# gabinsane/multimodal-vae-comparison

Measured on AMD Instinct MI355X. Metric: training samples/sec, MoPoE CdSprites+ L2 (fwd+bwd+Adam), higher is better.
Workload: dtype f32; 1 GPU; configs[1]: MoPoE, CdSprites+ L2 shapes, CNN2 image tower + TxtTransformer text tower, n_latents=32, batch=128/GPU, T=32; Adam(amsgrad) lr 1e-4, beta 1, train mode (dropout on); global_batch=128, parallelism=dp1, settle_steps=40

## Files before the change

include/mmvae_hip.h:

```cpp
#ifndef MMVAE_HIP_H
#define MMVAE_HIP_H

#include <stddef.h>
#include <stdint.h>

#ifdef __cplusplus
extern "C" {
#endif

typedef void* mmvae_stream_t;

enum {
  MMVAE_OK = 0,
  MMVAE_ERR_ARG = 1,
  MMVAE_ERR_UNSUPPORTED = 2,
  MMVAE_ERR_LAUNCH = 3
};

enum { MMVAE_ACT_NONE = 0, MMVAE_ACT_SILU = 1, MMVAE_ACT_RELU = 2, MMVAE_ACT_GELU = 3 };
enum {
  MMVAE_EP_NONE = 0,
  MMVAE_EP_RELU = 1,
  MMVAE_EP_MUL_RELU_MASK = 2,
  MMVAE_EP_MUL_SILU_GRAD = 3,
// ... 45 lines not shown
                           const mmvae_dropout_t* drop, const mmvae_dropout_t* ln_drop, mmvae_stream_t stream);
int mmvae_ffn32_bwd_b16(const float* x, const float* dy, const void* wsplit, const float* b1, float* dx, float* ws,
                        void* rsplit, const float* dx_add, int M, int FF, const mmvae_dropout_t* drop,
                        mmvae_stream_t stream);

int mmvae_version(void);
const char* mmvae_arch(void);


int mmvae_conv2d_k4s2_fwd(const float* x, const float* w, const float* bias, const float* aux, float* y,
                          int B, int Cin, int Cout, int Hin, int in_act, int ep_mode, mmvae_stream_t stream);

int mmvae_conv2d_k4s2_dgrad(const float* dy, const float* w, const float* aux, float* dx,
                            int B, int Cin, int Cout, int Hout, int ep_mode, mmvae_stream_t stream);

int mmvae_conv2d_k4s2_wgrad(const float* dy, const float* x, float* dw, float* db, float* ws,
                            int B, int Cin, int Cout, int Hout, int x_act, int accumulate, mmvae_stream_t stream);

int mmvae_convT2d_k4s2_fwd(const float* x, const float* w, const float* bias, const float* aux, float* y,
                           int B, int Cin, int Cout, int Hin, int in_act, int ep_mode, mmvae_stream_t stream);

int mmvae_convT2d_k4s2_dgrad(const float* dy, const float* w, const float* aux, float* dx,
                             int B, int Cin, int Cout, int Hin, int ep_mode, mmvae_stream_t stream);

int mmvae_convT2d_k4s2_wgrad(const float* x, const float* dy, float* dw, float* db, float* ws,
                             int B, int Cin, int Cout, int Hin, int x_act, int accumulate, mmvae_stream_t stream);

size_t mmvae_conv_wgrad_ws_floats(int B, int Csmall, int Clarge, int Hsmall);

int mmvae_conv2d_k4s2_bwd(const float* dy, const float* x, const float* w, float* dx, float* dw, float* db, float* ws,
                          int B, int Cin, int Cout, int Hout, int x_act, int accumulate, mmvae_stream_t stream);
int mmvae_convT2d_k4s2_bwd(const float* dy, const float* x, const float* w, float* dx, float* dw, float* db, float* ws,
                           int B, int Cin, int Cout, int Hin, int x_act, int accumulate, mmvae_stream_t stream);
int mmvae_convT3_bce_seeded(const float* x, const float* w, const float* bias, const float* target, float* row,
                            float* dlogit, float* part, unsigned* ticket, int B, int in_act, float seed,
                            mmvae_stream_t stream);
int mmvae_convT3_bce_strips(int B);
int mmvae_conv_plan(int split_bf16);

int mmvae_gemm_f32(const float* A, const float* Bm, const float* bias, const float* aux, float* C,
                   float* a_rowsum, float* ws, int M, int N, int K, long sam, long sak, long sbk, long sbn,
                   long ldc, int a_act, int b_act, int ep_mode, int accumulate, int splitk,
                   mmvae_stream_t stream);
size_t mmvae_gemm_ws_floats(int M, int N, int splitk);
int mmvae_gemm_splits(int M, int N, int K, int splitk);
int mmvae_gemm_b16_set(int on);
int mmvae_bias_group_add(float* y, const float* bias, int rows, int C, int G, mmvae_stream_t stream);
size_t mmvae_bias_group_ws_floats(int rows, int C);
int mmvae_bias_group_parts(int rows);
int mmvae_bias_group_grad(const float* dy, float* db, float* ws, int rows, int C, int G, int accumulate,
                          mmvae_stream_t stream);

int mmvae_linear_fwd(const float* x, const float* w, const float* b, float* aux, float* y, int M, int N, int K,
                     long ldx, int x_act, int ep_mode, mmvae_stream_t stream);
int mmvae_linear_bwd_data(const float* dy, const float* w, const float* aux, float* dx, int M, int N, int K,
                          int ep_mode, int accumulate, mmvae_stream_t stream);
int mmvae_linear_bwd_weight(const float* dy, const float* x, float* dw, float* db, float* ws, int M, int N, int K,
                            long ldx, int x_act, int accumulate, mmvae_stream_t stream);
size_t mmvae_linear_bwd_weight_ws_floats(int M, int N, int K);
#define MMVAE_WGRAD_BATCH_MAX 8
typedef struct {
  const float* dy; const float* x; float* dw; float* db; float* ws;
  int M, N, K; long ldx; int x_act, accumulate;
} mmvae_wgrad_job_t;
int mmvae_linear_bwd_weight_batch(const mmvae_wgrad_job_t* jobs, int n_jobs, mmvae_stream_t stream);
typedef struct {
// ... 487 lines not shown
```

multimodal_vae_comparison_amd/csrc/conv.hip:

```cpp
#include "conv_common.hpp"

#include "conv_gather.inc"
#include "conv_gather_b16.inc"
#include "conv_scatter.inc"
#include "conv_scatter_b16.inc"
#include "conv_wgrad.inc"

constexpr int cmax(int a, int b) { return a > b ? a : b; }

template <typename G, typename W, bool SPEC = false>
__global__ __launch_bounds__(256) void conv2d_bwd_fused_kernel(ConvScatterArgs ad, ConvWgradArgs aw, int n_w, int w_gx) {
  MMVAE_TRACE_STAMP(10 + G::LGH);
  __shared__ __attribute__((aligned(16))) float smem[cmax(G::SMEM, W::SMEM)];
  if ((int)blockIdx.x < n_w) conv_wgrad_body<W, SPEC>(aw, blockIdx.x % w_gx, blockIdx.x / w_gx, w_gx, smem);
  else
    conv_scatter_body<G>(ad, (n_w & 7) ? (int)blockIdx.x - n_w : xcd_contiguous(blockIdx.x - n_w, gridDim.x - n_w), smem);
}
template <typename G, typename W, bool SPEC = false>
__global__ __launch_bounds__(256) void convT_bwd_fused_kernel(ConvGatherArgs ad, ConvWgradArgs aw, int n_w, int w_gx) {
  MMVAE_TRACE_STAMP(14 - G::LGH);
  __shared__ __attribute__((aligned(16))) float smem[cmax(G::SMEM, W::SMEM)];
  if ((int)blockIdx.x < n_w) conv_wgrad_body<W, SPEC>(aw, blockIdx.x % w_gx, blockIdx.x / w_gx, w_gx, smem);
  else
    conv_gather_body<G, G::RWONLY>(ad, (n_w & 7) ? (int)blockIdx.x - n_w : xcd_contiguous(blockIdx.x - n_w, gridDim.x - n_w),
                                   smem);
}

template <typename GS, typename W, bool SPEC = false>
__global__ __launch_bounds__(256) void conv2d_bwd_fused_b16_kernel(ConvScatterArgs ad, ConvWgradArgs aw, int n_w, int w_gx) {
  MMVAE_TRACE_STAMP(10 + GS::LGH);
  __shared__ __attribute__((aligned(16))) unsigned char smem[cmax(GS::SMEM_TOTAL, 4 * W::SMEM)];
  if ((int)blockIdx.x < n_w)
    conv_wgrad_body<W, SPEC>(aw, blockIdx.x % w_gx, blockIdx.x / w_gx, w_gx, reinterpret_cast<float*>(smem));
  else
    conv_scatter_b16_body<GS, MMVAE_ACT_NONE>(
        ad, (n_w & 7) ? (int)blockIdx.x - n_w : xcd_contiguous(blockIdx.x - n_w, gridDim.x - n_w), 0, smem);
}

template <typename GB, typename W, bool SPEC = false>
__global__ __launch_bounds__(256) void convT_bwd_fused_b16_kernel(ConvGatherArgs ad, ConvWgradArgs aw, int n_w, int w_gx) {
  MMVAE_TRACE_STAMP(14 - GB::LGH);
  __shared__ __attribute__((aligned(16))) unsigned char smem[cmax(GB::SMEM_TOTAL, 4 * W::SMEM)];
  if ((int)blockIdx.x < n_w)
    conv_wgrad_body<W, SPEC>(aw, blockIdx.x % w_gx, blockIdx.x / w_gx, w_gx, reinterpret_cast<float*>(smem));
  else
    conv_gather_b16p_body<GB, MMVAE_ACT_NONE>(
        ad, (n_w & 7) ? (int)blockIdx.x - n_w : xcd_contiguous(blockIdx.x - n_w, gridDim.x - n_w), 0, smem);
}

// ... 43 lines not shown
        hipLaunchKernelGGL((conv2d_bwd_fused_b16_kernel<GS, W, true>), dim3(n_w + n_d), dim3(256), 0, st, ad, aw, n_w, nsplit);
      else
        hipLaunchKernelGGL((conv2d_bwd_fused_b16_kernel<GS, W>), dim3(n_w + n_d), dim3(256), 0, st, ad, aw, n_w, nsplit);
    };
    if (wgrad_qc8(nsplit, n_macro)) go(WgradGeom<32, 4, 8>{});
    else go(WgradGeom<32, 4>{});
    int rc0 = mmvae_launch_status();
    if (rc0) return rc0;
    return conv_bwd_reduce(ws, dw, db, B, Cin, Hout, 32, accumulate, stream);
  }
  scatter_visit(Hout, scatter_plan(tiles, 32, Hout), [&](auto g) {
    using G = decltype(g);
    if constexpr (G::LGH <= 4) {
      const int n_d = (int)scatter_grid(B, Hout, G::TM);
      if (wgrad_qc8(nsplit, n_macro)) {
        using W = WgradGeom<32, G::LGH, 8>;
        const int n_w = nsplit * W::NCH;
        if (wgrad_spec(n_macro, nsplit))
          hipLaunchKernelGGL((conv2d_bwd_fused_kernel<G, W, true>), dim3(n_w + n_d), dim3(256), 0, st, ad, aw, n_w, nsplit);
        else
          hipLaunchKernelGGL((conv2d_bwd_fused_kernel<G, W>), dim3(n_w + n_d), dim3(256), 0, st, ad, aw, n_w, nsplit);
      } else {
        using W = WgradGeom<32, G::LGH>;
        const int n_w = nsplit * W::NCH;
        hipLaunchKernelGGL((conv2d_bwd_fused_kernel<G, W>), dim3(n_w + n_d), dim3(256), 0, st, ad, aw, n_w, nsplit);
      }
      launched = true;
    }
  });
  if (!launched) return MMVAE_ERR_UNSUPPORTED;
  int rc = mmvae_launch_status();
  if (rc) return rc;
  return conv_bwd_reduce(ws, dw, db, B, Cin, Hout, 32, accumulate, stream);
}

extern "C" int mmvae_convT2d_k4s2_bwd(const float* dy, const float* x, const float* w, float* dx, float* dw, float* db,
                                      float* ws, int B, int Cin, int Cout, int Hin, int x_act, int accumulate,
                                      mmvae_stream_t stream) {
  MMVAE_CHECK_ARG(dy && x && w && dx && dw && ws && B > 0);
  hipStream_t st = (hipStream_t)stream;
  const int ep = dact_ep(x_act);
  const bool fused = Cin == 32 && (Cout == 32 || Cout == 3) && Hin >= 4 && Hin <= 32 && !(Hin & (Hin - 1)) &&
                     !(Cout == 3 && Hin != 32) && !(Cout == 32 && Hin > 16);
  if (!fused) {
    int rc = conv_wgrad_dispatch(x, dy, dw, db, ws, B, Cin, Cout, Hin, x_act, MMVAE_ACT_NONE, db ? 2 : 0, accumulate, st);
    if (rc) return rc;
    return conv_gather_dispatch(dy, w, nullptr, x, dx, B, Cout, Cin, 2 * Hin, MMVAE_ACT_NONE, ep, st);
  }
  ConvGatherArgs ad{dy, w, nullptr, x, dx, B, MMVAE_ACT_NONE, ep, CONV_CO};
  const long tiles = ((long)B * Hin * Hin + 31) / 32;
  const int n_macro = wgrad_n_macro(B, Hin), nsplit = wgrad_splits(n_macro, Cout);
  ConvWgradArgs aw{x, dy, ws, B, x_act, MMVAE_ACT_NONE, db ? 2 : 0, n_macro, 32, (long)32 * Cout * 16 + 32};
  bool launched = false;
  auto b16 = [&](auto gb) {
    using GB = decltype(gb);
    const int n_d = (int)((long)B * GB::HOUT / GB::NR);
    auto go = [&](auto wg) {
      using W = decltype(wg);
      const int n_w = nsplit * W::NCH;
      if (wgrad_spec(n_macro, nsplit))
        hipLaunchKernelGGL((convT_bwd_fused_b16_kernel<GB, W, true>), dim3(n_w + n_d), dim3(256), 0, st, ad, aw, n_w, nsplit);
      else
        hipLaunchKernelGGL((convT_bwd_fused_b16_kernel<GB, W>), dim3(n_w + n_d), dim3(256), 0, st, ad, aw, n_w, nsplit);
    };
    if constexpr (GB::CIN == 32) {
      if (wgrad_qc8(nsplit, n_macro)) go(WgradGeom<32, GB::LGH - 1, 8>{});
// ... 112 lines not shown
```

multimodal_vae_comparison_amd/csrc/conv_scatter.inc:

```
#include "conv_common.hpp"

struct ConvScatterArgs {
  const float* x;
  const float* w;
  const float* bias;
  const float* aux;
  float* y;
  int B, in_act, ep;
  int co_total;
};

template <int LGH_, int TM_, int CC_, int CIN_ = 32>
struct ScatterGeom {
  static constexpr int CIN = CIN_, LGH = LGH_, TM = TM_, CC = CC_;
  static constexpr int HIN = 1 << LGH, WIN = HIN, HOUT = 2 * HIN, WOUT = HOUT, LGW = LGH;
  static constexpr int RPT = WIN >= 32 ? 1 : 32 / WIN;
  static constexpr int NR = TM * RPT;
  static constexpr int NIMG = NR <= HIN ? 1 : NR / HIN;
  static constexpr int NROW = NR <= HIN ? NR : HIN;
  static constexpr int NRIN = NROW + 2;
  static constexpr int C0 = 4;
  static constexpr int RS = WIN == 16 ? 48 : WIN == 8 ? 40 : WIN == 4 ? 36 : 40;
  static constexpr int CS = NRIN * RS;
  static constexpr int IS0 = CC * CS;
  static constexpr int IS = (WIN == 4 && NIMG > 1) ? IS0 + ((16 - IS0 % 32 + 32) % 32) : IS0;
  static constexpr int KS = 4 / TM, CPW = CC / KS, NCHUNK = CIN / CC;
  static constexpr int RAW = NIMG * IS;
  static constexpr int IN_FLOATS = (KS > 1 && RAW < 4096) ? 4096 : (RAW + 3) / 4 * 4;
  static constexpr int SMEM = IN_FLOATS + CC * 16 * CONV_CO;
  static constexpr int F4ROW = WIN / 4, F4PP = NRIN * F4ROW;
  static constexpr int NF4 = NIMG * CC * F4PP;
  static constexpr int NSLOT = (NF4 + 255) / 256;
  static constexpr int WSLOT = CC * 4 * CONV_CO / 256;
  static_assert(CIN % CC == 0 && CC % KS == 0 && TM * KS == 4, "tile shape");
  static_assert(NSLOT <= 32, "validity mask");
};

template <typename G>
__device__ __forceinline__ void conv_scatter_body(const ConvScatterArgs& a, const int bid_x, float* __restrict__ smem,
                                                  const int og = 0) {
  constexpr int CIN = G::CIN, TM = G::TM, CC = G::CC, KS = G::KS, CPW = G::CPW;
  constexpr int HIN = G::HIN, WIN = G::WIN, HOUT = G::HOUT, WOUT = G::WOUT, LGW = G::LGW;
  constexpr int RS = G::RS, CS = G::CS;
  float* __restrict__ s_in = smem;
  float* __restrict__ s_w = smem + G::IN_FLOATS;

  const int tid = threadIdx.x, lane = tid & 63, wave = __builtin_amdgcn_readfirstlane(tid >> 6);
  const int li = lane & 31, lh = lane >> 5;
  const int tm = wave % TM, ks = wave / TM;
  const int Mtot = a.B * HIN * WIN;
  const int first_row = bid_x * G::NR;
  const int b0 = first_row >> LGW;
  const int h0 = G::NIMG > 1 ? 0 : first_row & (HIN - 1);

  int goff[G::NSLOT], lpos[G::NSLOT];
  unsigned svalid = 0;
#pragma unroll
  for (int s = 0; s < G::NSLOT; ++s) {
    const int q = tid + 256 * s;
    const int plane = q / G::F4PP, f = q - plane * G::F4PP;
    const int lr = f / G::F4ROW, c4 = f - lr * G::F4ROW;
    const int img = plane / CC, c = plane - img * CC;
    const int ih = h0 - 1 + lr;
    const bool ok = q < G::NF4 && ih >= 0 && ih < HIN && (b0 + img) < a.B;
    svalid |= (ok ? 1u : 0u) << s;
    goff[s] = ok ? ((img * CIN + c) * HIN + ih) * WIN + 4 * c4 : 0;
    lpos[s] = img * G::IS + c * CS + lr * RS + G::C0 + 4 * c4;
  }
  const float* xbase = a.x + (size_t)b0 * CIN * HIN * WIN;
  float4 rv[G::NSLOT], rw[G::WSLOT];
  auto load_chunk = [&](int ch) {
    const float* xch = xbase + (size_t)ch * CC * HIN * WIN;
#pragma unroll
// ... 12 lines not shown
      for (int s = 0; s < G::NSLOT; ++s) {
        rv[s].x = dev_silu(rv[s].x); rv[s].y = dev_silu(rv[s].y);
        rv[s].z = dev_silu(rv[s].z); rv[s].w = dev_silu(rv[s].w);
      }
    } else if (a.in_act == MMVAE_ACT_RELU) {
#pragma unroll
      for (int s = 0; s < G::NSLOT; ++s) {
        rv[s].x = fmaxf(rv[s].x, 0.f); rv[s].y = fmaxf(rv[s].y, 0.f);
        rv[s].z = fmaxf(rv[s].z, 0.f); rv[s].w = fmaxf(rv[s].w, 0.f);
      }
    }
#pragma unroll
    for (int s = 0; s < G::NSLOT; ++s) {
      if (tid + 256 * s < G::NF4) {
        const bool ok = svalid >> s & 1u;
        float4 o;
        o.x = ok ? rv[s].x : 0.f; o.y = ok ? rv[s].y : 0.f; o.z = ok ? rv[s].z : 0.f; o.w = ok ? rv[s].w : 0.f;
        *reinterpret_cast<float4*>(s_in + lpos[s]) = o;
      }
    }
#pragma unroll
    for (int i = 0; i < G::WSLOT; ++i) {
      const int e4 = i * 256 + tid;
      const int o = e4 & 31, kh = (e4 >> 5) & 3, cl = e4 >> 7;
      const int ph = 1 - (kh & 1), th = kh >> 1;
      float* d0 = s_w + ((((ph * 2 + 0) * CC + cl) * 2 + th) * 2) * CONV_CO + o;
      float* d1 = s_w + ((((ph * 2 + 1) * CC + cl) * 2 + th) * 2) * CONV_CO + o;
      d1[0] = rw[i].x;
      d0[0] = rw[i].y;
      d1[CONV_CO] = rw[i].z;
      d0[CONV_CO] = rw[i].w;
    }
  };

  load_chunk(0);
  for (int i = tid; i < G::NIMG * CC * G::NRIN * 2; i += 256) {
    const int side = i & 1, r = i >> 1;
    const int plane = r / G::NRIN, lr = r - plane * G::NRIN;
    const int img = plane / CC, c = plane - img * CC;
    s_in[img * G::IS + c * CS + lr * RS + G::C0 - 1 + side * (WIN + 1)] = 0.f;
  }

  const int tile_p0 = (bid_x * TM + tm) * 32;
  int abase;
  {
    int p = tile_p0 + li;
    if (p > Mtot - 1) p = Mtot - 1;
    const int R = p >> LGW, s = p & (WIN - 1);
    int rl = R - first_row;
    if (rl < 0) rl = 0;
    const int img_l = G::NIMG > 1 ? rl >> LGW : 0;
    const int r_l = G::NIMG > 1 ? rl & (HIN - 1) : rl;
    abase = img_l * G::IS + (r_l + 1) * RS + (s + G::C0 - lh) + ks * CPW * CS;
  }
  const int wbase = (ks * CPW * 4 + lh) * CONV_CO + li;

  f32x16 acc[4];
#pragma unroll
  for (int c = 0; c < 4; ++c)
#pragma unroll
    for (int r = 0; r < 16; ++r) acc[c][r] = 0.f;

#pragma unroll 1
  for (int ch = 0; ch < G::NCHUNK; ++ch) {
    if (ch > 0) __syncthreads();
    store_chunk();
    __syncthreads();
    if (ch + 1 < G::NCHUNK) load_chunk(ch + 1);
    {
      float av[2][6], bv[2][8];
      auto load_ops = [&](int cc, int buf) {
#pragma unroll
        for (int dr = 0; dr < 3; ++dr)
#pragma unroll
          for (int pw = 0; pw < 2; ++pw) av[buf][dr * 2 + pw] = s_in[abase + cc * CS + (dr - 1) * RS + pw];
#pragma unroll
        for (int cls = 0; cls < 4; ++cls)
#pragma unroll
          for (int th = 0; th < 2; ++th) bv[buf][cls * 2 + th] = s_w[wbase + (((cls * CC + cc) * 2 + th) * 2) * CONV_CO];
      };
      load_ops(0, 0);
#pragma unroll
      for (int cc = 0; cc < CPW; ++cc) {
        if (cc + 1 < CPW) load_ops(cc + 1, (cc + 1) & 1);
        __builtin_amdgcn_sched_barrier(0);
#pragma unroll
        for (int cls = 0; cls < 4; ++cls)
#pragma unroll
          for (int th = 0; th < 2; ++th) {
            const int ph = cls >> 1, pw = cls & 1;
            acc[cls] = __builtin_amdgcn_mfma_f32_32x32x2f32(av[cc & 1][(ph - th + 1) * 2 + pw], bv[cc & 1][cls * 2 + th],
                                                            acc[cls], 0, 0, 0);
          }
        __builtin_amdgcn_sched_barrier(0);
      }
    }
  }

  const float bias = a.bias ? a.bias[og * CONV_CO + li] : 0.f;
  auto store8 = [&](int q, int ph, const float* e0, const float* e1) {
    const int p0 = tile_p0 + 8 * q + 4 * lh;
    if (p0 < Mtot) {
      const int R = p0 >> LGW, s = p0 & (WIN - 1);
      const int b = R >> LGW, r = R & (HIN - 1);
      const size_t off = (((size_t)b * a.co_total + og * CONV_CO + li) * HOUT + 2 * r + ph) * WOUT + 2 * s;
      float4 o0 = make_float4(e0[0] + bias, e1[0] + bias, e0[1] + bias, e1[1] + bias);
      float4 o1 = make_float4(e0[2] + bias, e1[2] + bias, e0[3] + bias, e1[3] + bias);
      if (a.ep != MMVAE_EP_NONE) {
        float4 a0 = make_float4(0.f, 0.f, 0.f, 0.f), a1 = a0;
        if (ep_reads_aux(a.ep)) {
          a0 = *reinterpret_cast<const float4*>(a.aux + off);
          a1 = *reinterpret_cast<const float4*>(a.aux + off + 4);
        }
        o0.x = conv_epilogue(o0.x, a0.x, a.ep); o0.y = conv_epilogue(o0.y, a0.y, a.ep);
        o0.z = conv_epilogue(o0.z, a0.z, a.ep); o0.w = conv_epilogue(o0.w, a0.w, a.ep);
        o1.x = conv_epilogue(o1.x, a1.x, a.ep); o1.y = conv_epilogue(o1.y, a1.y, a.ep);
        o1.z = conv_epilogue(o1.z, a1.z, a.ep); o1.w = conv_epilogue(o1.w, a1.w, a.ep);
      }
      *reinterpret_cast<float4*>(a.y + off) = o0;
      *reinterpret_cast<float4*>(a.y + off + 4) = o1;
    }
  };

  if (KS == 1) {
#pragma unroll
    for (int ph = 0; ph < 2; ++ph)
#pragma unroll
      for (int q = 0; q < 4; ++q) {
        float e0[4], e1[4];
#pragma unroll
        for (int e = 0; e < 4; ++e) {
          e0[e] = acc[ph * 2 + 0][4 * q + e];
          e1[e] = acc[ph * 2 + 1][4 * q + e];
        }
        store8(q, ph, e0, e1);
      }
  } else {
    float* red = s_in;
#pragma unroll
    for (int ph = 0; ph < 2; ++ph) {
      float sum[2][4 / KS][4];
#pragma unroll
      for (int pw = 0; pw < 2; ++pw) {
        __syncthreads();
#pragma unroll
        for (int r = 0; r < 16; ++r) red[(wave * 16 + r) * 64 + lane] = acc[ph * 2 + pw][r];
        __syncthreads();
#pragma unroll
        for (int qq = 0; qq < 4 / KS; ++qq) {
          const int q = ks * (4 / KS) + qq;
#pragma unroll
          for (int e = 0; e < 4; ++e) {
            float s = 0.f;
#pragma unroll
            for (int k2 = 0; k2 < KS; ++k2) s += red[((k2 * TM + tm) * 16 + 4 * q + e) * 64 + lane];
            sum[pw][qq][e] = s;
          }
        }
      }
#pragma unroll
      for (int qq = 0; qq < 4 / KS; ++qq) store8(ks * (4 / KS) + qq, ph, sum[0][qq], sum[1][qq]);
    }
  }
}

struct ConvScatter3Args {
  const float* x;
  const float* w;
  const float* bias;
  float* y;
  int B, in_act, ep;
};

template <int LGH_, int NT_ = 2>
struct Scatter3Geom {
  static constexpr int CIN = 32, CO = 3, LGH = LGH_;
  static constexpr int NT = NT_;
  static constexpr int POS = 64 * NT;
  static constexpr int HIN = 1 << LGH, WIN = HIN, HOUT = 2 * HIN, WOUT = HOUT;
  static constexpr int NR = POS / WIN;
  static constexpr int NRIN = NR + 2;
  static constexpr int C0 = 4;
  static constexpr int RS = (WIN + 5 + 3) / 4 * 4;
  static constexpr int CS0 = NRIN * RS;
  static constexpr int CS = CS0 + ((16 - CS0 % 32 + 32) % 32);
  static constexpr int IN_FLOATS = CIN * CS;
  static constexpr int SMEM = IN_FLOATS + 9 * CIN * 16;
  static constexpr int F4ROW = WIN / 4, F4PP = NRIN * F4ROW, NF4 = CIN * F4PP, NSLOT = (NF4 + 255) / 256;
  static_assert(NR >= 1 && NR <= HIN, "one image per workgroup");
};

template <typename G>
__device__ __forceinline__ void conv_scatter3_body(const ConvScatter3Args& a, const int bid_x, float* __restrict__ smem) {
  constexpr int CIN = G::CIN, CO = G::CO, HIN = G::HIN, WIN = G::WIN, HOUT = G::HOUT, WOUT = G::WOUT;
  constexpr int RS = G::RS, CS = G::CS;
// ... 210 lines not shown
```

multimodal_vae_comparison_amd/hipops.py:

```python
import ctypes
import os

import torch

_HERE = os.path.dirname(os.path.abspath(__file__))
LIB_PATH = os.path.join(_HERE, "libmmvae_hip.so")
_lib = None

c_p = ctypes.c_void_p
c_i = ctypes.c_int
c_l = ctypes.c_long
c_f = ctypes.c_float
c_u = ctypes.c_uint
c_sz = ctypes.c_size_t

MAX_EXPERTS = 8

ACT_NONE, ACT_SILU, ACT_RELU, ACT_GELU = 0, 1, 2, 3
EP_NONE, EP_RELU, EP_MUL_RELU_MASK, EP_MUL_SILU_GRAD, EP_GELU, EP_MUL_GELU_GRAD, EP_SIGMOID_CLAMP, EP_SIGMOID, EP_ADD_AUX = range(9)

_ERR = {1: "invalid argument", 2: "unsupported shape", 3: "kernel launch failed"}


class PoeFwdArgs(ctypes.Structure):
# ... 69 lines not shown
                ("mY", c_p), ("mmean", c_p), ("msc", c_p), ("mbeta", c_p), ("out", c_p), ("ws", c_p), ("tile_ticket", c_p),
                ("row_map", c_p), ("M", c_i), ("Min", c_i), ("Cin", c_i), ("Cout", c_i), ("T", c_i), ("nstat", c_i), ("g", RcGeom),
                ("st", RcStat * 2)]


class RcWgrad(ctypes.Structure):
    _fields_ = [("G", c_p), ("Y", c_p), ("pqr", c_p), ("x", c_p), ("xmean", c_p), ("xsc", c_p), ("xbeta", c_p), ("tbl", c_p),
                ("dw", c_p), ("ws", c_p), ("counter", c_p), ("M", c_i), ("Cin", c_i), ("Cout", c_i), ("T", c_i), ("pre", c_i),
                ("accumulate", c_i)]


RC_MAX_JOBS = 8


class RcJob(ctypes.Structure):
    _fields_ = [("kind", c_i), ("f", RcFwd), ("d", RcDgrad), ("w", RcWgrad)]


c_dp = ctypes.POINTER(Dropout)
DROPOUT_SLOTS = 16

SIGNATURES = {
    "mmvae_version": (c_i, []),
    "mmvae_arch": (ctypes.c_char_p, []),
    "mmvae_conv2d_k4s2_fwd": (c_i, [c_p] * 5 + [c_i] * 6 + [c_p]),
    "mmvae_conv2d_k4s2_dgrad": (c_i, [c_p] * 4 + [c_i] * 5 + [c_p]),
    "mmvae_conv2d_k4s2_wgrad": (c_i, [c_p] * 5 + [c_i] * 6 + [c_p]),
    "mmvae_convT2d_k4s2_fwd": (c_i, [c_p] * 5 + [c_i] * 6 + [c_p]),
    "mmvae_convT2d_k4s2_dgrad": (c_i, [c_p] * 4 + [c_i] * 5 + [c_p]),
    "mmvae_convT2d_k4s2_wgrad": (c_i, [c_p] * 5 + [c_i] * 6 + [c_p]),
    "mmvae_conv_wgrad_ws_floats": (c_sz, [c_i] * 4),
    "mmvae_conv2d_k4s2_bwd": (c_i, [c_p] * 7 + [c_i] * 6 + [c_p]),
    "mmvae_convT2d_k4s2_bwd": (c_i, [c_p] * 7 + [c_i] * 6 + [c_p]),
    "mmvae_gemm_f32": (c_i, [c_p] * 7 + [c_i] * 3 + [c_l] * 5 + [c_i] * 5 + [c_p]),
    "mmvae_gemm_ws_floats": (c_sz, [c_i] * 3),
    "mmvae_gemm_splits": (c_i, [c_i] * 4),
    "mmvae_bias_group_add": (c_i, [c_p, c_p, c_i, c_i, c_i, c_p]),
    "mmvae_bias_group_grad": (c_i, [c_p, c_p, c_p, c_i, c_i, c_i, c_i, c_p]),
    "mmvae_bias_group_ws_floats": (c_sz, [c_i, c_i]),
    "mmvae_bias_group_parts": (c_i, [c_i]),
    "mmvae_linear_fwd": (c_i, [c_p] * 5 + [c_i] * 3 + [c_l] + [c_i] * 2 + [c_p]),
    "mmvae_gemm_b16_set": (c_i, [c_i]),
    "mmvae_attn_t_bwd_set": (c_i, [c_i]),
    "mmvae_linear_bwd_data": (c_i, [c_p] * 4 + [c_i] * 5 + [c_p]),
    "mmvae_linear_bwd_weight": (c_i, [c_p] * 5 + [c_i] * 3 + [c_l] + [c_i] * 2 + [c_p]),
    "mmvae_linear_bwd_weight_ws_floats": (c_sz, [c_i] * 3),
    "mmvae_linear_bwd_weight_batch": (c_i, [c_p, c_i, c_p]),
    "mmvae_txt_layer_plan": (c_i, [c_i] * 3),
    "mmvae_conv_plan": (c_i, [c_i]),
    "mmvae_convT3_bce_seeded": (c_i, [c_p] * 8 + [c_i, c_i, c_f, c_p]),
    "mmvae_convT3_bce_strips": (c_i, [c_i]),
    "mmvae_txt_wgrad": (c_i, [c_p, c_i, c_p]),
    "mmvae_txt_wgrad_splits": (c_i, [c_i] * 3),
    "mmvae_txt_wgrad_ws_floats": (c_sz, [c_i] * 3),
    "mmvae_txt_wgrad_supported": (c_i, [c_i] * 3),
    "mmvae_input_pipe_create": (c_i, [c_p, c_p, c_sz]),
    "mmvae_input_pipe_destroy": (c_i, [c_p]),
    "mmvae_input_pipe_prefetch": (c_i, [c_p, c_p]),
    "mmvae_input_pipe_commit": (c_i, [c_p, c_p, c_i, c_p, c_p]),
    "mmvae_linear_bwd": (c_i, [c_p] * 8 + [c_i] * 3 + [c_l] + [c_i] * 3 + [c_p]),
    "mmvae_linear_bwd_ws_floats": (c_sz, [c_i] * 3),
    "mmvae_head_softmax_fwd": (c_i, [c_p, c_i, c_i, c_p]),
    "mmvae_head_softmax_bwd": (c_i, [c_p, c_p, c_i, c_i, c_p]),
    "mmvae_poe_reparam_kl_fwd": (c_i, [ctypes.POINTER(PoeFwdArgs), c_p, c_p, c_p, c_i, c_i, c_i, c_u, c_i, c_i, c_i,
                                       c_i, c_p, c_p]),
    "mmvae_poe_reparam_kl_bwd": (c_i, [ctypes.POINTER(PoeBwdArgs), c_p, c_p, c_p, c_p, c_p, c_i, c_i, c_i, c_u, c_i, c_i,
# ... 261 lines not shown
```

multimodal_vae_comparison_amd/models/encoders.py:

```python
import os

import numpy as np
import torch
import torch.nn as nn

from .. import hipops as H
from .. import ops
from .NetworkTypes import NetworkRoles, NetworkTypes
from .nn_modules import DropoutState, HipLayerNorm, HipLinear, HipSelfAttention, ModuleWrap, PositionalEncoding


class VaeComponent(nn.Module):

    def __init__(self, latent_dim, data_dim, latent_private=None, enc_mu_logvar=True,
                 net_type=NetworkTypes.UNSPECIFIED, net_role=NetworkRoles.UNSPECIFIED):
        super().__init__()
        self.net_role = net_role
        self.latent_dim = latent_dim
        self.enc_mu_logvar = enc_mu_logvar
        self.latent_private = latent_private
        self.out_dim = latent_dim + latent_private if latent_private is not None else latent_dim
        self.data_dim = data_dim
        self.net_type = net_type
        self.mu_layer = None
# ... 60 lines not shown

    def __init__(self, cin, cout, in_act=H.ACT_NONE):
        super().__init__()
        ref = nn.Conv2d(cin, cout, 4, stride=2, padding=1)
        self.weight, self.bias = ref.weight, ref.bias
        self.in_act = in_act

    def flat_groups(self):
        return [[self.weight, self.bias]]

    def forward(self, x):
        return ops.conv2d_k4s2(x, self.weight, self.bias, self.in_act, self.weight.grad, self.bias.grad)


class Enc_CNN2(VaeEncoder):

    def __init__(self, latent_dim, data_dim, latent_private, enc_mu_logvar):
        data_dim = (3, 64, 64)
        super().__init__(latent_dim, data_dim, latent_private, enc_mu_logvar, net_type=NetworkTypes.CNN)
        hid = 32
        self.hidden_dim = 512
        self.reshape = (hid, 4, 4)
        self.conv1 = HipConv2d(3, hid, H.ACT_NONE)
        self.conv2 = HipConv2d(hid, hid, H.ACT_SILU)
        self.conv3 = HipConv2d(hid, hid, H.ACT_SILU)
        self.conv4 = HipConv2d(hid, hid, H.ACT_SILU)
        self.lin1 = HipLinear(int(np.prod(self.reshape)), self.hidden_dim, H.ACT_SILU)
        self.init_final_layers(self.hidden_dim)

    def forward(self, x):
        if isinstance(x, dict):
            x = x["data"]
        bs = x.size(0)
        u = self.conv4(self.conv3(self.conv2(self.conv1(x.float()))))
        o5 = self.lin1(u.view(bs, -1))
        return self.process_output(o5)


class HipConv(nn.Module):

    def __init__(self, cin, cout, k, stride, pad, in_act=H.ACT_NONE, transposed=False, out_ep=H.EP_NONE):
        super().__init__()
        ref = (nn.ConvTranspose2d if transposed else nn.Conv2d)(cin, cout, k, stride=stride, padding=pad)
        self.weight, self.bias = ref.weight, ref.bias
        self.cfg = (stride, pad, in_act, transposed, out_ep)

    def flat_groups(self):
        return [[self.weight, self.bias]]

    def forward(self, x, ep_bwd=True):
        stride, pad, in_act, transposed, out_ep = self.cfg
        if transposed:
            return ops.convT2d(x, self.weight, self.bias, stride, pad, in_act, out_ep, self.weight.grad, self.bias.grad,
                               ep_bwd)
        return ops.conv2d(x, self.weight, self.bias, stride, pad, in_act, self.weight.grad, self.bias.grad)


class _HiddenHeads:

    def _heads(self):
        return self.hidden_mu, self.hidden_logvar


class Enc_MNIST(_HiddenHeads, VaeEncoder):

    def __init__(self, latent_dim, data_dim, latent_private, enc_mu_logvar):
        super().__init__(latent_dim, data_dim, latent_private, enc_mu_logvar, net_type=NetworkTypes.FNN)
# ... 279 lines not shown
```

multimodal_vae_comparison_amd/ops.py:

```python
import bisect
import ctypes
import os

import torch
from torch.autograd import Function

from . import hipops as H

_DACT = {H.ACT_NONE: H.EP_NONE, H.ACT_SILU: H.EP_MUL_SILU_GRAD, H.ACT_RELU: H.EP_MUL_RELU_MASK,
         H.ACT_GELU: H.EP_MUL_GELU_GRAD}


CALLS = [0]


def _call(name, *args):
    CALLS[0] += 1
    H.check(getattr(H.lib(), name)(*args), name)


class GradReducer:

    enabled = True
    tail = None
# ... 460 lines not shown
        x, w = ctx.saved_tensors
        in_act, gw, gb, has_b = ctx.cfg
        dy = H.f32c(dy)
        B, Cin, Hin, _ = x.shape
        Cout, Hout = w.shape[0], Hin // 2
        dw, acc_w, ret_w = _new_like_param(w, gw)
        db, ret_b = None, None
        if has_b:
            if gb is not None:
                db = gb
            else:
                db = ret_b = torch.empty(Cout, device=x.device)
        nws = H.lib().mmvae_conv_wgrad_ws_floats(B, Cout, Cin, Hout)
        defer = _defer(gw, gb if has_b else gw)
        ws = GradReducer.alloc(nws, x.device) if defer else H.workspace(nws, x.device)
        acc = H.ACC_DEFER if defer else acc_w
        dx = None
        if ctx.needs_input_grad[0]:
            dx = torch.empty_like(x)
            _call("mmvae_conv2d_k4s2_bwd", H.ptr(dy), H.ptr(x), H.ptr(w), H.ptr(dx), H.ptr(dw), H.ptr(db), H.ptr(ws),
                  B, Cin, Cout, Hout, in_act, acc, H.stream())
        else:
            def launch(dy=dy, x=x, dw=dw, db=db, ws=ws):
                _call("mmvae_conv2d_k4s2_wgrad", H.ptr(dy), H.ptr(x), H.ptr(dw), H.ptr(db), H.ptr(ws), B, Cin, Cout,
                      Hout, in_act, acc, H.stream())
            if defer and StreamPlan.enabled and StreamPlan.batch_wgrad:
                GradReducer.queue(x.device, launch, dy, x)
            else:
                with torch.cuda.stream(_wgrad_side(x.device, dy, x) if defer else None):
                    launch()
        if defer:
            _conv_segments(ws, dw, db, B, Cout, Cin, Hout, Cout)
        return dx, ret_w, ret_b, None, None, None


class ConvT2dK4S2(Function):

    @staticmethod
    def forward(ctx, x, w, b, in_act, out_ep, gw, gb, ep_bwd=True):
        x = H.f32c(x)
        B, Cin, Hin, _ = x.shape
        Cout = w.shape[1]
        y = torch.empty(B, Cout, 2 * Hin, 2 * Hin, device=x.device, dtype=torch.float32)
        _call("mmvae_convT2d_k4s2_fwd", H.ptr(x), H.ptr(w), H.ptr(b), None, H.ptr(y), B, Cin, Cout, Hin, in_act,
              out_ep, H.stream())
        if not ep_bwd:
            out_ep = H.EP_NONE
        ctx.save_for_backward(x, w, y if out_ep in (H.EP_SIGMOID_CLAMP, H.EP_SIGMOID) else None)
        ctx.cfg = (in_act, out_ep, gw, gb, b is not None)
        return y

    @staticmethod
    def backward(ctx, dy):
        x, w, y = ctx.saved_tensors
        in_act, out_ep, gw, gb, has_b = ctx.cfg
        dy = H.f32c(dy)
        B, Cin, Hin, _ = x.shape
        Cout = w.shape[1]
        if out_ep == H.EP_SIGMOID_CLAMP:
            dl = torch.empty_like(dy)
            _call("mmvae_sigmoid_clamp_bwd", H.ptr(dy), H.ptr(y), H.ptr(dl), dy.numel(), H.stream())
            dy = dl
        elif out_ep == H.EP_SIGMOID:
            dl = torch.empty_like(dy)
            _call("mmvae_sigmoid_bwd", H.ptr(dy), H.ptr(y), H.ptr(dl), dy.numel(), H.stream())
            dy = dl
# ... 2277 lines not shown
```

Before: 335,600 samples/s.

## Fuse first conv layer weight-grad into second conv's backward data-grad kernel

In the image encoder, conv1 and conv2 are now run as one autograd function. In its backward, conv2's input-gradient tile is never written to global memory. The scatter kernel instead loads the matching input-image patch into shared memory and uses MFMA to accumulate conv1's weight and bias gradients in registers. Per-block partial rows are reduced afterwards or handed to the deferred GradReducer. This removes the dx round trip for conv1 and one wgrad launch, at the cost of extra register and shared-memory pressure (launch bounds 256,3) and a narrow shape-gated path.

Result: no change. 337,100 samples/s, median of 2 (+0.4%).

```diff
diff --git a/include/mmvae_hip.h b/include/mmvae_hip.h
--- a/include/mmvae_hip.h
+++ b/include/mmvae_hip.h
@@ -101,6 +101,10 @@
                           int B, int Cin, int Cout, int Hout, int x_act, int accumulate, mmvae_stream_t stream);
 int mmvae_convT2d_k4s2_bwd(const float* dy, const float* x, const float* w, float* dx, float* dw, float* db, float* ws,
                            int B, int Cin, int Cout, int Hin, int x_act, int accumulate, mmvae_stream_t stream);
+int mmvae_conv2d_k4s2_bwd_first(const float* dy, const float* x, const float* w, const float* img, float* dw, float* db,
+                                float* ws, float* dw0, float* db0, float* ws0, int B, int Cin, int Cout, int Hout,
+                                int x_act, int accumulate, mmvae_stream_t stream);
+int mmvae_conv2d_bwd_first_layout(int B, int* rows, int* rowlen, int* bias_col);
 int mmvae_convT3_bce_seeded(const float* x, const float* w, const float* bias, const float* target, float* row,
                             float* dlogit, float* part, unsigned* ticket, int B, int in_act, float seed,
                             mmvae_stream_t stream);
diff --git a/multimodal_vae_comparison_amd/csrc/conv.hip b/multimodal_vae_comparison_amd/csrc/conv.hip
--- a/multimodal_vae_comparison_amd/csrc/conv.hip
+++ b/multimodal_vae_comparison_amd/csrc/conv.hip
@@ -15,6 +15,16 @@
   if ((int)blockIdx.x < n_w) conv_wgrad_body<W, SPEC>(aw, blockIdx.x % w_gx, blockIdx.x / w_gx, w_gx, smem);
   else
     conv_scatter_body<G>(ad, (n_w & 7) ? (int)blockIdx.x - n_w : xcd_contiguous(blockIdx.x - n_w, gridDim.x - n_w), smem);
+}
+template <typename G, typename W>
+__global__ __launch_bounds__(256, 3) void conv2d_bwd_first_kernel(ConvScatterArgs ad, ConvWgradArgs aw, ConvFirstArgs af, int n_w,
+                                                               int w_gx) {
+  MMVAE_TRACE_STAMP(10 + G::LGH);
+  __shared__ __attribute__((aligned(16))) float smem[cmax(G::SMEM, W::SMEM)];
+  if ((int)blockIdx.x < n_w) conv_wgrad_body<W>(aw, blockIdx.x % w_gx, blockIdx.x / w_gx, w_gx, smem);
+  else
+    conv_scatter_body<G, true>(ad, (n_w & 7) ? (int)blockIdx.x - n_w : xcd_contiguous(blockIdx.x - n_w, gridDim.x - n_w), smem,
+                               0, &af);
 }
 template <typename G, typename W, bool SPEC = false>
 __global__ __launch_bounds__(256) void convT_bwd_fused_kernel(ConvGatherArgs ad, ConvWgradArgs aw, int n_w, int w_gx) {
@@ -124,6 +134,44 @@
   int rc = mmvae_launch_status();
   if (rc) return rc;
   return conv_bwd_reduce(ws, dw, db, B, Cin, Hout, 32, accumulate, stream);
+}
+
+using FirstG = ScatterGeom<4, 2, 8, 32>;
+using FirstW = WgradGeom<32, 4, 8>;
+static inline int first_rows(int B) { return (int)scatter_grid(B, 16, FirstG::TM); }
+extern "C" int mmvae_conv2d_k4s2_bwd_first(const float* dy, const float* x, const float* w, const float* img, float* dw,
+                                           float* db, float* ws, float* dw0, float* db0, float* ws0, int B, int Cin,
+                                           int Cout, int Hout, int x_act, int accumulate, mmvae_stream_t stream) {
+  MMVAE_CHECK_ARG(dy && x && w && img && dw && ws && dw0 && ws0 && B > 0);
+  hipStream_t st = (hipStream_t)stream;
+  const long tiles = ((long)B * Hout * Hout + 31) / 32;
+  if (Cin != 32 || Cout != 32 || Hout != 16 || tiles >= 2048) return MMVAE_ERR_UNSUPPORTED;
+  const int ep = dact_ep(x_act);
+  if (!conv_ep_supported(ep)) return MMVAE_ERR_UNSUPPORTED;
+  const int n_macro = wgrad_n_macro(B, Hout), nsplit = wgrad_splits(n_macro, 32);
+  if (!wgrad_qc8(nsplit, n_macro) || wgrad_spec(n_macro, nsplit)) return MMVAE_ERR_UNSUPPORTED;
+  ConvScatterArgs ad{dy, w, nullptr, x, nullptr, B, MMVAE_ACT_NONE, ep, CONV_CO};
+  ConvWgradArgs aw{dy, x, ws, B, MMVAE_ACT_NONE, x_act, db ? 1 : 0, n_macro, 32, (long)32 * 32 * 16 + 32};
+  ConvFirstArgs af{img, ws0};
+  const int n_w = nsplit * FirstW::NCH, n_d = first_rows(B);
+  hipLaunchKernelGGL((conv2d_bwd_first_kernel<FirstG, FirstW>), dim3(n_w + n_d), dim3(256), 0, st, ad, aw, af, n_w, nsplit);
+  int rc = mmvae_launch_status();
+  if (rc) return rc;
+  rc = conv_bwd_reduce(ws, dw, db, B, Cin, Hout, 32, accumulate, stream);
+  if (rc || accumulate == MMVAE_ACC_DEFER) return rc;
+  using FG = FirstGeom<FirstG>;
+  rc = mmvae_reduce_rows(ws0, dw0, n_d, FG::DWLEN, FG::ROWLEN, accumulate, stream);
+  if (rc) return rc;
+  if (db0) rc = mmvae_reduce_rows(ws0 + FG::DWLEN, db0, n_d, CONV_CO, FG::ROWLEN, accumulate, stream);
+  return rc;
+}
+extern "C" int mmvae_conv2d_bwd_first_layout(int B, int* rows, int* rowlen, int* bias_col) {
+  MMVAE_CHECK_ARG(rows && rowlen && bias_col && B > 0);
+  using FG = FirstGeom<FirstG>;
+  *rows = first_rows(B);
+  *rowlen = FG::ROWLEN;
+  *bias_col = FG::DWLEN;
+  return MMVAE_OK;
 }
 
 extern "C" int mmvae_convT2d_k4s2_bwd(const float* dy, const float* x, const float* w, float* dx, float* dw, float* db,
diff --git a/multimodal_vae_comparison_amd/csrc/conv_scatter.inc b/multimodal_vae_comparison_amd/csrc/conv_scatter.inc
--- a/multimodal_vae_comparison_amd/csrc/conv_scatter.inc
+++ b/multimodal_vae_comparison_amd/csrc/conv_scatter.inc
@@ -1,3 +1,5 @@
+#include <type_traits>
+
 #include "conv_common.hpp"
 
 struct ConvScatterArgs {
@@ -36,9 +38,29 @@
   static_assert(NSLOT <= 32, "validity mask");
 };
 
+struct ConvFirstArgs {
+  const float* img;
+  float* ws;
+};
 template <typename G>
+struct FirstGeom {
+  static constexpr int Q = 3, IH = 2 * G::HOUT, IW = IH;
+  static constexpr int NRIN = 4 * G::NR + 2;
+  static constexpr int C0 = 4, RS = IW + 4;
+  static constexpr int CS0 = NRIN * RS + 4;
+  static constexpr int CS = CS0 + ((16 - CS0 % 32 + 32) % 32);
+  static constexpr int FLOATS = Q * CS;
+  static constexpr int F4ROW = IW / 4, F4PP = NRIN * F4ROW, NF4 = Q * F4PP, NSLOT = (NF4 + 255) / 256;
+  static constexpr int DWLEN = CONV_CO * Q * 16, ROWLEN = DWLEN + CONV_CO;
+  static_assert(G::KS > 1 && G::NIMG == 1 && G::WIN >= 8 && G::CIN == 32, "written for the K-split tile shapes");
+  static_assert(FLOATS <= G::CC * 16 * CONV_CO, "the patch takes the weight tile's place");
+  static_assert(4 * ROWLEN <= G::SMEM, "cross-wave sum");
+  static_assert(RS % 32 == 4, "bank layout");
+};
+
+template <typename G, bool FIRST = false>
 __device__ __forceinline__ void conv_scatter_body(const ConvScatterArgs& a, const int bid_x, float* __restrict__ smem,
-                                                  const int og = 0) {
+                                                  const int og = 0, const ConvFirstArgs* fa = nullptr) {
   constexpr int CIN = G::CIN, TM = G::TM, CC = G::CC, KS = G::KS, CPW = G::CPW;
   constexpr int HIN = G::HIN, WIN = G::WIN, HOUT = G::HOUT, WOUT = G::WOUT, LGW = G::LGW;
   constexpr int RS = G::RS, CS = G::CS;
@@ -117,6 +139,47 @@
       d0[CONV_CO] = rw[i].w;
     }
   };
+
+  using FG = FirstGeom<std::conditional_t<FIRST, G, ScatterGeom<4, 2, 8, 32>>>;
+  float* s_p = s_w;
+  float4 pv[FIRST ? FG::NSLOT : 1];
+  unsigned pvalid = 0;
+  auto load_patch = [&]() {
+    const float* ib = fa->img + (size_t)b0 * FG::Q * FG::IH * FG::IW;
+#pragma unroll
+    for (int s = 0; s < FG::NSLOT; ++s) {
+      const int q = tid + 256 * s;
+      const int c = q / FG::F4PP, f = q - c * FG::F4PP;
+      const int lr = f / FG::F4ROW, c4 = f - lr * FG::F4ROW;
+      const int ih = 4 * h0 - 1 + lr;
+      const bool ok = q < FG::NF4 && ih >= 0 && ih < FG::IH;
+      pvalid |= (ok ? 1u : 0u) << s;
+      pv[s] = *reinterpret_cast<const float4*>(ib + (ok ? (c * FG::IH + ih) * FG::IW + 4 * c4 : 0));
+    }
+  };
+  auto store_patch = [&]() {
+#pragma unroll
+    for (int s = 0; s < FG::NSLOT; ++s) {
+      const int q = tid + 256 * s;
+      if (q < FG::NF4) {
+        const int c = q / FG::F4PP, f = q - c * FG::F4PP;
+        const int lr = f / FG::F4ROW, c4 = f - lr * FG::F4ROW;
+        const bool ok = pvalid >> s & 1u;
+        float4 o;
+        o.x = ok ? pv[s].x : 0.f; o.y = ok ? pv[s].y : 0.f; o.z = ok ? pv[s].z : 0.f; o.w = ok ? pv[s].w : 0.f;
+        *reinterpret_cast<float4*>(s_p + c * FG::CS + lr * FG::RS + FG::C0 + 4 * c4) = o;
+      }
+    }
+    for (int i = tid; i < FG::Q * FG::NRIN * 2; i += 256) {
+      const int side = i & 1, r = i >> 1;
+      const int c = r / FG::NRIN, lr = r - c * FG::NRIN;
+      s_p[c * FG::CS + lr * FG::RS + FG::C0 - 1 + side * (FG::IW + 1)] = 0.f;
+    }
+  };
+  f32x16 wacc[FIRST ? 2 : 1];
+  float fsum = 0.f;
+  const int pb0 = (li >> 4) * FG::CS + ((li >> 2) & 3) * FG::RS + (li & 3) + (FG::C0 - 1) + lh * 16;
+  const int pb1 = 2 * FG::CS + ((li >> 2) & 3) * FG::RS + (li & 3) + (FG::C0 - 1) + lh * 16;
 
   load_chunk(0);
   for (int i = tid; i < G::NIMG * CC * G::NRIN * 2; i += 256) {
@@ -146,42 +209,56 @@
 #pragma unroll
     for (int r = 0; r < 16; ++r) acc[c][r] = 0.f;
 
+  auto mma_chunk = [&]() {
+    float av[2][6], bv[2][8];
+    auto load_ops = [&](int cc, int buf) {
+#pragma unroll
+      for (int dr = 0; dr < 3; ++dr)
+#pragma unroll
+        for (int pw = 0; pw < 2; ++pw) av[buf][dr * 2 + pw] = s_in[abase + cc * CS + (dr - 1) * RS + pw];
+#pragma unroll
+      for (int cls = 0; cls < 4; ++cls)
+#pragma unroll
+        for (int th = 0; th < 2; ++th) bv[buf][cls * 2 + th] = s_w[wbase + (((cls * CC + cc) * 2 + th) * 2) * CONV_CO];
+    };
+    load_ops(0, 0);
+#pragma unroll
+    for (int cc = 0; cc < CPW; ++cc) {
+      if (cc + 1 < CPW) load_ops(cc + 1, (cc + 1) & 1);
+      __builtin_amdgcn_sched_barrier(0);
+#pragma unroll
+      for (int cls = 0; cls < 4; ++cls)
+#pragma unroll
+        for (int th = 0; th < 2; ++th) {
+          const int ph = cls >> 1, pw = cls & 1;
+          acc[cls] = __builtin_amdgcn_mfma_f32_32x32x2f32(av[cc & 1][(ph - th + 1) * 2 + pw], bv[cc & 1][cls * 2 + th],
+                                                          acc[cls], 0, 0, 0);
+        }
+      __builtin_amdgcn_sched_barrier(0);
+    }
+  };
 #pragma unroll 1
-  for (int ch = 0; ch < G::NCHUNK; ++ch) {
+  for (int ch = 0; ch < G::NCHUNK - (FIRST ? 1 : 0); ++ch) {
     if (ch > 0) __syncthreads();
     store_chunk();
     __syncthreads();
     if (ch + 1 < G::NCHUNK) load_chunk(ch + 1);
-    {
-      float av[2][6], bv[2][8];
-      auto load_ops = [&](int cc, int buf) {
-#pragma unroll
-        for (int dr = 0; dr < 3; ++dr)
-#pragma unroll
-          for (int pw = 0; pw < 2; ++pw) av[buf][dr * 2 + pw] = s_in[abase + cc * CS + (dr - 1) * RS + pw];
-#pragma unroll
-        for (int cls = 0; cls < 4; ++cls)
-#pragma unroll
-          for (int th = 0; th < 2; ++th) bv[buf][cls * 2 + th] = s_w[wbase + (((cls * CC + cc) * 2 + th) * 2) * CONV_CO];
-      };
-      load_ops(0, 0);
-#pragma unroll
-      for (int cc = 0; cc < CPW; ++cc) {
-        if (cc + 1 < CPW) load_ops(cc + 1, (cc + 1) & 1);
-        __builtin_amdgcn_sched_barrier(0);
-#pragma unroll
-        for (int cls = 0; cls < 4; ++cls)
-#pragma unroll
-          for (int th = 0; th < 2; ++th) {
-            const int ph = cls >> 1, pw = cls & 1;
-            acc[cls] = __builtin_amdgcn_mfma_f32_32x32x2f32(av[cc & 1][(ph - th + 1) * 2 + pw], bv[cc & 1][cls * 2 + th],
-                                                            acc[cls], 0, 0, 0);
-          }
-        __builtin_amdgcn_sched_barrier(0);
-      }
-    }
-  }
-
+    mma_chunk();
+  }
+  if constexpr (FIRST) {
+    if (G::NCHUNK > 1) __syncthreads();
+    store_chunk();
+    __syncthreads();
+    load_patch();
+    mma_chunk();
+  }
+
+  if constexpr (FIRST) {
+#pragma unroll
+    for (int n = 0; n < 2; ++n)
+#pragma unroll
+      for (int r = 0; r < 16; ++r) wacc[n][r] = 0.f;
+  }
   const float bias = a.bias ? a.bias[og * CONV_CO + li] : 0.f;
   auto store8 = [&](int q, int ph, const float* e0, const float* e1) {
     const int p0 = tile_p0 + 8 * q + 4 * lh;
@@ -202,8 +279,26 @@
         o1.x = conv_epilogue(o1.x, a1.x, a.ep); o1.y = conv_epilogue(o1.y, a1.y, a.ep);
         o1.z = conv_epilogue(o1.z, a1.z, a.ep); o1.w = conv_epilogue(o1.w, a1.w, a.ep);
       }
-      *reinterpret_cast<float4*>(a.y + off) = o0;
-      *reinterpret_cast<float4*>(a.y + off + 4) = o1;
+      if constexpr (FIRST) {
+        const int rl = R - first_row;
+        const int po = 2 * (2 * rl + ph) * FG::RS + 4 * ((8 * q) & (WIN - 1));
+        const float v[8] = {o0.x, o0.y, o0.z, o0.w, o1.x, o1.y, o1.z, o1.w};
+        float b0v[8], b1v[8];
+#pragma unroll
+        for (int j = 0; j < 8; ++j) {
+          b0v[j] = s_p[pb0 + po + 2 * j];
+          b1v[j] = s_p[pb1 + po + 2 * j];
+        }
+#pragma unroll
+        for (int j = 0; j < 8; ++j) {
+          fsum += v[j];
+          wacc[0] = __builtin_amdgcn_mfma_f32_32x32x2f32(v[j], b0v[j], wacc[0], 0, 0, 0);
+          wacc[1] = __builtin_amdgcn_mfma_f32_32x32x2f32(v[j], b1v[j], wacc[1], 0, 0, 0);
+        }
+      } else {
+        *reinterpret_cast<float4*>(a.y + off) = o0;
+        *reinterpret_cast<float4*>(a.y + off + 4) = o1;
+      }
     }
   };
 
@@ -228,6 +323,9 @@
 #pragma unroll
       for (int pw = 0; pw < 2; ++pw) {
         __syncthreads();
+        if constexpr (FIRST) {
+          if (ph == 0 && pw == 0) store_patch();
+        }
 #pragma unroll
         for (int r = 0; r < 16; ++r) red[(wave * 16 + r) * 64 + lane] = acc[ph * 2 + pw][r];
         __syncthreads();
@@ -246,6 +344,22 @@
 #pragma unroll
       for (int qq = 0; qq < 4 / KS; ++qq) store8(ks * (4 / KS) + qq, ph, sum[0][qq], sum[1][qq]);
     }
+  }
+  if constexpr (FIRST) {
+    __syncthreads();
+    float* mine = smem + wave * FG::ROWLEN;
+#pragma unroll
+    for (int n = 0; n < 2; ++n)
+      if (n * 32 + li < FG::Q * 16) {
+#pragma unroll
+        for (int r = 0; r < 16; ++r) mine[((r & 3) + 8 * (r >> 2) + 4 * lh) * (FG::Q * 16) + n * 32 + li] = wacc[n][r];
+      }
+    const float fs = fsum + __shfl_xor(fsum, 32, 64);
+    if (lh == 0) mine[FG::DWLEN + li] = fs;
+    __syncthreads();
+    float* row = fa->ws + (size_t)bid_x * FG::ROWLEN;
+    for (int i = tid; i < FG::ROWLEN; i += 256)
+      row[i] = ((smem[i] + smem[FG::ROWLEN + i]) + smem[2 * FG::ROWLEN + i]) + smem[3 * FG::ROWLEN + i];
   }
 }
 
diff --git a/multimodal_vae_comparison_amd/hipops.py b/multimodal_vae_comparison_amd/hipops.py
--- a/multimodal_vae_comparison_amd/hipops.py
+++ b/multimodal_vae_comparison_amd/hipops.py
@@ -125,6 +125,8 @@
     "mmvae_conv_wgrad_ws_floats": (c_sz, [c_i] * 4),
     "mmvae_conv2d_k4s2_bwd": (c_i, [c_p] * 7 + [c_i] * 6 + [c_p]),
     "mmvae_convT2d_k4s2_bwd": (c_i, [c_p] * 7 + [c_i] * 6 + [c_p]),
+    "mmvae_conv2d_k4s2_bwd_first": (c_i, [c_p] * 10 + [c_i] * 6 + [c_p]),
+    "mmvae_conv2d_bwd_first_layout": (c_i, [c_i] + [c_p] * 3),
     "mmvae_gemm_f32": (c_i, [c_p] * 7 + [c_i] * 3 + [c_l] * 5 + [c_i] * 5 + [c_p]),
     "mmvae_gemm_ws_floats": (c_sz, [c_i] * 3),
     "mmvae_gemm_splits": (c_i, [c_i] * 4),
diff --git a/multimodal_vae_comparison_amd/models/encoders.py b/multimodal_vae_comparison_amd/models/encoders.py
--- a/multimodal_vae_comparison_amd/models/encoders.py
+++ b/multimodal_vae_comparison_amd/models/encoders.py
@@ -116,7 +116,14 @@
         if isinstance(x, dict):
             x = x["data"]
         bs = x.size(0)
-        u = self.conv4(self.conv3(self.conv2(self.conv1(x.float()))))
+        x = x.float()
+        c1, c2 = self.conv1, self.conv2
+        grads = (c1.weight.grad, c1.bias.grad, c2.weight.grad, c2.bias.grad)
+        if ops.conv_first_fused_ok(x, c1.weight, c1.bias, c2.weight, c2.bias, *grads):
+            u = ops.conv2d_k4s2_first(x, c1.weight, c1.bias, c2.weight, c2.bias, c2.in_act, *grads)
+        else:
+            u = c2(c1(x))
+        u = self.conv4(self.conv3(u))
         o5 = self.lin1(u.view(bs, -1))
         return self.process_output(o5)
 
diff --git a/multimodal_vae_comparison_amd/ops.py b/multimodal_vae_comparison_amd/ops.py
--- a/multimodal_vae_comparison_amd/ops.py
+++ b/multimodal_vae_comparison_amd/ops.py
@@ -516,6 +516,76 @@
         if defer:
             _conv_segments(ws, dw, db, B, Cout, Cin, Hout, Cout)
         return dx, ret_w, ret_b, None, None, None
+
+
+CONV_FIRST_FUSED = os.environ.get("MMVAE_CONV_FIRST_FUSED", "1") == "1"
+_first_layouts = {}
+
+
+def conv_first_fused_ok(img, w1, b1, w2, b2, gw1, gb1, gw2, gb2):
+    if not (CONV_FIRST_FUSED and img.is_cuda and img.dim() == 4 and not img.requires_grad):
+        return False
+    B = img.shape[0]
+    return (tuple(img.shape[1:]) == (3, 64, 64) and tuple(w1.shape) == (32, 3, 4, 4) and tuple(w2.shape) == (32, 32, 4, 4)
+            and b1 is not None and b2 is not None and 64 <= B < 256
+            and len({g is None for g in (gw1, gb1, gw2, gb2)}) == 1)
+
+
+class Conv2dK4S2First(Function):
+
+    @staticmethod
+    def forward(ctx, img, w1, b1, w2, b2, act2, gw1, gb1, gw2, gb2):
+        img = H.f32c(img)
+        B, _, Hin, _ = img.shape
+        y1 = torch.empty(B, 32, Hin // 2, Hin // 2, device=img.device, dtype=torch.float32)
+        _call("mmvae_conv2d_k4s2_fwd", H.ptr(img), H.ptr(w1), H.ptr(b1), None, H.ptr(y1), B, 3, 32, Hin, H.ACT_NONE,
+              H.EP_NONE, H.stream())
+        y2 = torch.empty(B, 32, Hin // 4, Hin // 4, device=img.device, dtype=torch.float32)
+        _call("mmvae_conv2d_k4s2_fwd", H.ptr(y1), H.ptr(w2), H.ptr(b2), None, H.ptr(y2), B, 32, 32, Hin // 2, act2,
+              H.EP_NONE, H.stream())
+        ctx.save_for_backward(img, y1, w1, w2)
+        ctx.cfg = (act2, gw1, gb1, gw2, gb2)
+        return y2
+
+    @staticmethod
+    def backward(ctx, dy):
+        img, y1, w1, w2 = ctx.saved_tensors
+        act2, gw1, gb1, gw2, gb2 = ctx.cfg
+        dy = H.f32c(dy)
+        B, Hout = img.shape[0], img.shape[-1] // 4
+        dw2, acc, ret_w2 = _new_like_param(w2, gw2)
+        dw1, _, ret_w1 = _new_like_param(w1, gw1)
+        db2, db1 = gb2, gb1
+        ret_b2 = ret_b1 = None
+        if gb2 is None:
+            db2, db1 = torch.empty(32, device=img.device), torch.empty(32, device=img.device)
+            ret_b2, ret_b1 = db2, db1
+        lay = _first_layouts.get(B)
+        if lay is None:
+            rows, rowlen, bias_col = ctypes.c_int(), ctypes.c_int(), ctypes.c_int()
+            H.check(H.lib().mmvae_conv2d_bwd_first_layout(B, ctypes.byref(rows), ctypes.byref(rowlen), ctypes.byref(bias_col)),
+                    "mmvae_conv2d_bwd_first_layout")
+            lay = _first_layouts[B] = (rows.value, rowlen.value, bias_col.value)
+        rows, rowlen, bias_col = lay
+        nws = H.lib().mmvae_conv_wgrad_ws_floats(B, 32, 32, Hout)
+        defer = _defer(gw1, gb1, gw2, gb2)
+        if defer:
+            ws, ws0 = GradReducer.alloc(nws, img.device), GradReducer.alloc(rows * rowlen, img.device)
+            acc = H.ACC_DEFER
+        else:
+            both = H.workspace(nws + rows * rowlen, img.device)
+            ws, ws0 = both[:nws], both[nws:]
+        _call("mmvae_conv2d_k4s2_bwd_first", H.ptr(dy), H.ptr(y1), H.ptr(w2), H.ptr(img), H.ptr(dw2), H.ptr(db2), H.ptr(ws),
+              H.ptr(dw1), H.ptr(db1), H.ptr(ws0), B, 32, 32, Hout, act2, acc, H.stream())
+        if defer:
+            _conv_segments(ws, dw2, db2, B, 32, 32, Hout, 32)
+            GradReducer.add(ws0.data_ptr(), dw1, rows, dw1.numel(), rowlen)
+            GradReducer.add(ws0.data_ptr() + 4 * bias_col, db1, rows, 32, rowlen)
+        return None, ret_w1, ret_b1, ret_w2, ret_b2, None, None, None, None, None
+
+
+def conv2d_k4s2_first(img, w1, b1, w2, b2, act2, gw1=None, gb1=None, gw2=None, gb2=None):
+    return Conv2dK4S2First.apply(img, w1, b1, w2, b2, act2, gw1, gb1, gw2, gb2)
 
 
 class ConvT2dK4S2(Function):
```
